# amidos2006/gym-pcgrl

Measured on AMD Instinct MI355X. Metric: env-steps/sec (whole node), binary-narrow 14x14 @ 65536 envs, higher is better.
Workload: dtype u8; 1 GPU; binary-narrow-v0 14x14, 65536 envs/GPU; envs_per_gpu=65536, width=14, height=14, max_changes=39, actions=uniform random, device-generated before the timed region, parallelism=env-axis shard x1, no collective on the step path

## Files before the change

gym_pcgrl_amd/csrc/kernels_stats.h:

```cpp
#pragma once
template <class MaskT>
__device__ __forceinline__ MaskT row_valid(int lane, int W, int H) {
    MaskT full = (W >= (int)(8 * sizeof(MaskT))) ? ~(MaskT)0 : (((MaskT)1 << W) - 1);
    return lane < H ? full : (MaskT)0;
}

template <int PROB = -1>
__device__ __forceinline__ bool finalize_item(const PcgrlParams& P, const DevBufs& B, int e, const int32_t* s,
                                              int mode, int parity, int shard, bool push_reset = true, int rst_list = WL_RST,
                                              const int2* pre = nullptr, const double* reward_pre = nullptr) {
    const int prob = PROB >= 0 ? PROB : P.prob;
    int32_t* st = B.stats + (size_t)e * 8;
    int32_t* start = B.start_stats + (size_t)e * 8;
    if (mode == MODE_STEP) {
        int32_t old[PCGRL_MAX_STATS], sv[PCGRL_MAX_STATS];
        for (int k = 0; k < 8; k++) { old[k] = st[k]; sv[k] = start[k]; }
        const int2 c = pre ? *pre : reinterpret_cast<const int2*>(B.counters)[e];
        const double r = reward_pre ? *reward_pre : compute_reward(P, s, old, prob);
        const bool d = episode_over(P, s, sv, prob) || c.y >= P.max_changes || c.x >= P.max_iterations;
        B.reward[e] = r;
        B.done[e] = d ? 1 : 0;
        episode_account(B, e, r, d);
        int32_t* inf = B.info + (size_t)e * 10;
#pragma unroll
// ... 48 lines not shown
        int32_t* park = (mode == MODE_STEP) ? B.info + (size_t)e * 10 : B.stats + (size_t)e * 8;
        for (int k = 0; k < 8; k++) park[k] = s[k];
        wl_push(B, parity, park_list >= 0 ? park_list : (mode == MODE_STEP ? WL_SOL : WL_SOL2), shard, e);
        return false;
    }
    return finalize_item<PROB>(P, B, e, s, mode, parity, shard, push_reset, WL_RST, nullptr, reward_pre);
}

template <int J>
__device__ __forceinline__ double dpp_down(double v) {
    const long long b = __double_as_longlong(v);
    const int lo = __builtin_amdgcn_update_dpp(0, (int)b, 0x100 + J, 0xF, 0xF, true), hi = __builtin_amdgcn_update_dpp(0, (int)(b >> 32), 0x100 + J, 0xF, 0xF, true);
    return __longlong_as_double(((long long)hi << 32) | (unsigned)lo);
}
__device__ __forceinline__ void zelda_reward_tab(const PcgrlParams& P, ZeldaRewardTab* T) {
    T->w[0] = P.rewards[0]; T->w[1] = P.rewards[1]; T->w[2] = P.rewards[2]; T->w[3] = P.rewards[4]; T->w[4] = P.rewards[3];
    T->w[5] = P.rewards[5]; T->w[6] = P.rewards[6]; T->w[7] = 0.0;
    T->lo[0] = 1; T->lo[1] = 1; T->lo[2] = 1; T->lo[3] = 2; T->lo[4] = 1; T->lo[5] = P.target_enemy_dist; T->lo[6] = PCGRL_IPOS; T->lo[7] = 0;
    T->hi[0] = 1; T->hi[1] = 1; T->hi[2] = 1; T->hi[3] = P.max_enemies; T->hi[4] = 1; T->hi[5] = PCGRL_IPOS; T->hi[6] = PCGRL_IPOS; T->hi[7] = 0;
}
__device__ __forceinline__ double zelda_reward_lanes(const ZeldaRewardTab* T, const int32_t* old, const int32_t* s, int k) {
    const int s0 = s[0], s1 = s[1], s2 = s[2], s3 = s[3], s4 = s[4], s5 = s[5], s6 = s[6];
    int n = s6;
    n = k == 5 ? s5 : n; n = k == 4 ? s4 : n; n = k == 3 ? s3 : n; n = k == 2 ? s2 : n; n = k == 1 ? s1 : n; n = k == 0 ? s0 : n;
    const int kk = k & 7;
    const int o = old[kk];
    const double t = k < 7 ? (double)range_reward_i(n, o, T->lo[kk], T->hi[kk]) * T->w[kk] : 0.0;
    double r = t;
    r = r + dpp_down<1>(t); r = r + dpp_down<2>(t); r = r + dpp_down<3>(t);
    r = r + dpp_down<4>(t); r = r + dpp_down<5>(t); r = r + dpp_down<6>(t);
    return r;
}

template <int PROB, int G, class MaskT, bool FUSED = false>
__device__ __forceinline__ void stats_wave_task(const PcgrlParams& P, const DevBufs& B, DevGroup<G, MaskT>& g, int lane64, int gw, bool lone,
                                                bool inc, bool pair, bool zinc, bool have, int raw, int shard, int mode, int parity,
                                                int inline_reset, int gen_map, uint32_t* mt, uint8_t* tiles, MaskT rowmask,
                                                StepLocal* SL = nullptr, bool step_obs = false) {
    constexpr bool kCanReset = PROB == PCGRL_PROB_BINARY || PROB == PCGRL_PROB_ZELDA;
    if (!kCanReset) inline_reset = 0;
    constexpr int GPW = 64 / G;
    constexpr bool kInc = PROB == PCGRL_PROB_BINARY;
    constexpr bool kZinc = PROB == PCGRL_PROB_ZELDA && G == 16 && sizeof(MaskT) == 4;
    constexpr int NPL = (PROB == PCGRL_PROB_BINARY) ? 1 : 3;
    MaskT* champ_base = reinterpret_cast<MaskT*>(B.champ);
    const bool tch = kInc && G == 16 && !inc && !lone && have && raw < 0;
    const bool packed = inc || (kZinc && zinc && !lone) || tch;
    const bool reset_only = have && !packed && (raw & WL_RESET_ONLY) != 0;
    const bool compute = have && !reset_only && !(lone && (gw & 1));
    const int e = packed ? wl_inc_env<G>(raw) : (raw & ~WL_RESET_ONLY);
    MaskT* planes_e = reinterpret_cast<MaskT*>(B.planes) + (size_t)e * NPL * G;
    MaskT b0 = 0, b1 = 0, b2 = 0;
    if (compute) {
        b0 = planes_e[g.lane * NPL];
        if (NPL > 1) { b1 = planes_e[g.lane * NPL + 1]; b2 = planes_e[g.lane * NPL + 2]; }
    }
    if (GPW >= 2 && lone && inline_reset) {
        const int role = gw & 1;
        int2 pre = make_int2(0, 0);
        if (g.lane == 0 && role == 0 && have) pre = reinterpret_cast<const int2*>(B.counters)[e];
        asm volatile("s_waitcnt vmcnt(0)" ::: "memory");
#pragma unroll
        for (int k = 0; k < GPW / 2; k++) {
            if (k > 0 && !pair) break;
            if (!__builtin_amdgcn_readlane((int)have, 2 * k * G)) continue;
            const int ek = __builtin_amdgcn_readlane(e, 2 * k * G);
            const int step_draws = (SL && P.rep == PCGRL_REP_NARROW && P.random_tile) ? 1 : 0;
            if (SL && lane64 == 0) SL->dirty[ek - SL->e0] = 1;
            ResetRows rr;
            wave_reset_env<PROB, !FUSED, FUSED>(P, B, ek, gen_map, mt, (uint8_t*)nullptr, lane64, step_draws, gw == 2 * k + 1 ? g.lane : -1, &rr);
            MaskT t0, t1, t2;
// ... 48 lines not shown
    } else {
        bool full = compute;
        if (kInc && G == 16) {
            const bool t = compute && tch;
            if (t) {
                const MaskT cbit = (g.lane == wl_inc_row<G>(raw)) ? (MaskT)1 << wl_inc_col<G>(raw) : (MaskT)0;
                const MaskT champ_old = champ_base[(size_t)e * G + g.lane];
                const int4 old = *reinterpret_cast<const int4*>(B.stats + (size_t)e * 8);
                int regions, path, ub2;
                if (binary_touch(g, (MaskT)(~b0 & rowmask), cbit, (wl_inc_code<G>(raw) & 1u) != 0, old.x, champ_old, old.w - 1, regions, path, champ, ub2)) {
                    s[0] = regions; s[1] = path; s[2] = 1; s[3] = ub2 + 1;
                    full = false;
                }
            }
        }
        if (full) need_solver = compute_item_stats<PROB>(g, P, b0, b1, b2, rowmask, s, champ, (B.step_tight & 1) != 0);
    }
    if (kInc && compute && champ_base) champ_base[(size_t)e * G + g.lane] = champ;
    TL(10);
    int want_reset = 0;
    constexpr bool kLaneReward = PROB == PCGRL_PROB_ZELDA && G == 16;
    double rpre = 0.0;
    const bool lane_reward = kLaneReward && SL != nullptr && mode == MODE_STEP;
    if (lane_reward && have && !reset_only) rpre = zelda_reward_lanes(&SL->zr, B.stats + (size_t)e * 8, s, g.lane);
    if (g.lane == 0 && have) {
        if (reset_only) want_reset = 1;
        else want_reset = finish_or_park<PROB>(P, B, e, s, need_solver, mode, parity, shard, !inline_reset, -1, lane_reward ? &rpre : nullptr) ? 1 : 0;
    }
    if (inline_reset) {
        const uint64_t want = __ballot(want_reset != 0);
        TL(11);
        if (want) {
            TL(12);
            if (SL) { while (__hip_atomic_load(&SL->refill_done[SL->par], __ATOMIC_ACQUIRE, __HIP_MEMORY_SCOPE_WORKGROUP) < SL->need) __builtin_amdgcn_s_sleep(2); }
            bool mine = false;
#pragma unroll
            for (int k = 0; k < GPW; k++) {
                if ((want >> (k * G)) & 1ull) {
                    const int ek = __builtin_amdgcn_readlane(e, k * G);
                    if (SL && lane64 == 0) { SL->dirty[ek - SL->e0] = 1; SL->late[ek - SL->e0] = 1; SL->n_late = 1; }
                    int pend = 0;
                    if (SL) {
                        if (lane64 == 0) {
                            pend = atomicExch(&SL->pend[ek - SL->e0], 0);
                            if (pend < 0) {
                                while (__hip_atomic_load(&SL->late_done[(ek - SL->e0) >> 6], __ATOMIC_ACQUIRE, __HIP_MEMORY_SCOPE_WORKGROUP) == 0) __builtin_amdgcn_s_sleep(2);
                                pend = 0;
                            }
                        }
                        pend = __builtin_amdgcn_readfirstlane(pend);
                    }
                    ResetRows rr;
                    wave_reset_env<PROB, !FUSED, FUSED>(P, B, ek, gen_map, mt, (uint8_t*)nullptr, lane64, 0, gw == k ? g.lane : -1, &rr, pend);
                    MaskT t0, t1, t2;
                    reset_rows_to_planes<MaskT>(P, reinterpret_cast<MaskT*>(B.planes) + (size_t)ek * NPL * G, gw == k ? g.lane : -1, rr.m0, rr.m1, rr.m2, t0, t1, t2);
                    if (gw == k) { b0 = t0; b1 = t1; b2 = t2; mine = true; }
                    __builtin_amdgcn_wave_barrier();
                }
            }
            if (mine) {
                int32_t st[PCGRL_MAX_STATS] = {0, 0, 0, 0, 0, 0, 0, 0};
                const bool ns = compute_item_stats<PROB>(g, P, b0, b1, b2, rowmask, st, champ, (B.step_tight & 2) != 0);
                if (kInc && champ_base) champ_base[(size_t)e * G + g.lane] = champ;
                if (g.lane == 0) finish_or_park<PROB>(P, B, e, st, ns, MODE_START, parity, shard);
            }
        }
    }
// ... 316 lines not shown
```

gym_pcgrl_amd/csrc/kernels_step.h:

```cpp
#pragma once

struct StepLds { int planes, champ, stats, start, cnt, cur, fifo, tag, pos, act, flat, in_total, info, rew, done, total; };
__host__ __device__ constexpr StepLds step_lds_layout(int plane_row_bytes, int champ_row_bytes, bool fifo, int action_width, int epb) {
    StepLds L = {};
    int o = 0;
    L.planes = o; o += epb * plane_row_bytes;
    L.champ = o; o += epb * champ_row_bytes;
    L.stats = o; o += epb * 32;
    L.start = o; o += epb * 32;
    L.cnt = o; o += epb * 8;
    L.cur = o; o += epb * 8;
    L.fifo = o; o += fifo ? epb * PCGRL_FIFO_N * 4 : 0;
    L.tag = o; o += fifo ? epb * 4 : 0;
    L.pos = o; o += epb * 2;
    L.act = o; o += epb * 4 * action_width;
    L.flat = o; o += action_width == 3 ? epb * 4 : 0;
    L.in_total = o;
    L.info = o; o += epb * 40;
    L.rew = o; o += epb * 8;
    L.done = o; o += epb;
    L.total = (o + 15) & ~15;
    return L;
}

// ... 129 lines not shown
            PCGRL_SEG_LOAD(L.tag / 16, EPB / 4, has_fifo ? Bg.fifo_tag + e0 : nullptr, has_fifo);
        }
        PCGRL_SEG_LOAD(L.pos / 16, EPB / 8, Bg.pos + (size_t)e0 * 2, true);
        if (!ROW) PCGRL_SEG_LOAD(L.act / 16, EPB / 4 * AW, actions + (size_t)e0 * AW, !(AW == 3 && Bg.flat));
        if (!ROW && AW == 3) PCGRL_SEG_LOAD(L.flat / 16, (AW == 3 ? EPB / 4 : 1), Bg.flat ? Bg.flat + e0 : nullptr, Bg.flat != nullptr);
        asm volatile("" ::: "memory");
        static_assert(L.act % 16 == 0, "the prefetch ends on a slot boundary in front of the actions");
        constexpr int TOT = (ROW ? L.act : L.in_total) / 16;
        seg_store_c<TPB, 0, TOT>(smem, r0, tid0); seg_store_c<TPB, 1, TOT>(smem, r1, tid0); seg_store_c<TPB, 2, TOT>(smem, r2, tid0);
        seg_store_c<TPB, 3, TOT>(smem, r3, tid0); seg_store_c<TPB, 4, TOT>(smem, r4, tid0); seg_store_c<TPB, 5, TOT>(smem, r5, tid0);
        seg_store_c<TPB, 6, TOT>(smem, r6, tid0); seg_store_c<TPB, 7, TOT>(smem, r7, tid0); seg_store_c<TPB, 8, TOT>(smem, r8, tid0);
    } else {
        blk_copy<TPB>(smem + L.planes, g_planes, ne * kPlaneRow);
        if (has_champ) blk_copy<TPB>(smem + L.champ, g_champ, ne * champ_row);
        blk_copy<TPB>(smem + L.stats, reinterpret_cast<const uint8_t*>(Bg.stats + (size_t)e0 * 8), ne * 32);
        blk_copy<TPB>(smem + L.start, reinterpret_cast<const uint8_t*>(Bg.start_stats + (size_t)e0 * 8), ne * 32);
        blk_copy<TPB>(smem + L.cnt, reinterpret_cast<const uint8_t*>(Bg.counters + (size_t)e0 * 2), ne * 8);
        blk_copy<TPB>(smem + L.cur, reinterpret_cast<const uint8_t*>(Bg.rng_cur + (size_t)e0 * 2), ne * 8);
        blk_copy<TPB>(smem + L.pos, Bg.pos + (size_t)e0 * 2, ne * 2);
        if (has_fifo) {
            blk_copy<TPB>(smem + L.fifo, reinterpret_cast<const uint8_t*>(Bg.fifo + (size_t)e0 * PCGRL_FIFO_N), ne * PCGRL_FIFO_N * 4);
            blk_copy<TPB>(smem + L.tag, reinterpret_cast<const uint8_t*>(Bg.fifo_tag + e0), ne * 4);
        }
        if (ROW) {}
        else if (AW == 3 && Bg.flat) blk_copy<TPB>(smem + L.flat, reinterpret_cast<const uint8_t*>(Bg.flat + e0), ne * 4);
        else blk_copy<TPB>(smem + L.act, reinterpret_cast<const uint8_t*>(actions + (size_t)e0 * AW), ne * 4 * AW);
    }
    if (row_have) {
        reinterpret_cast<int32_t*>(smem + (row_fl ? L.flat : L.act))[threadIdx.x] = (int32_t)row_act;
        if (Bg.row.actions_out) Bg.row.actions_out[row_a0] = row_act;
    }
    if (threadIdx.x < EPB) { s_loc.dirty[threadIdx.x] = 0; if (OBS) { s_loc.obs_skip[threadIdx.x] = 0; s_loc.late[threadIdx.x] = 0; } }
    if (threadIdx.x < 8) s_n[threadIdx.x >> 2][threadIdx.x & 3] = 0;
    if (threadIdx.x == 0) { s_loc.e0 = 0; s_loc.need = NUPD; s_loc.refill_done[0] = 0; s_loc.refill_done[1] = 0; s_loc.n_late = 0; s_obs_ticket = 0; }
    constexpr int OBS_PER_TASK = 8;
    const bool obs_delta = OBS && REP == PCGRL_REP_WIDE && NPL == 3 && Bg.obs.delta;
    const int n_obs = (OBS && !obs_delta) ? (ne + OBS_PER_TASK - 1) / OBS_PER_TASK : 0;
    const ObsPlanes<MaskT, NPL> obs_src = {reinterpret_cast<const MaskT*>(smem + L.planes), G};
    if (OBS && threadIdx.x == 0) s_loc.obs_v = obs_view(P, Bg.obs, e0);
    if (PROB == PCGRL_PROB_ZELDA && threadIdx.x == 64) zelda_reward_tab(P, &s_loc.zr);
    uint8_t* reset_scratch = smem + L.total;
#pragma clang loop unroll(disable)
  for (int t = 0; t < (MULTI ? steps : 1); t++) {
    int tid = (int)threadIdx.x;
    if (MULTI) asm volatile("" : "+v"(tid));
    const int lane64 = tid & 63, wv = tid >> 6, gw = lane64 / G;
    const int sp = t & 1;
    DevGroup<G, MaskT> g(lane64);
    if (MULTI && t > 0) {
        const int32_t* row = actions + (size_t)t * action_stride + (size_t)e0 * AW;
        for (int i = tid; i < ne * AW; i += TPB) reinterpret_cast<int32_t*>(smem + L.act)[i] = row[i];
    }
    __syncthreads();
    TL(17);
    const int prio = B.step_prio, prio_nfull = (prio >> 8) & 15;
    int prio_now = 0;
    if (wv < NUPD) {
        if ((prio >> 6) & 3) { prio_now = (prio >> 6) & 3; step_set_prio(prio_now); }
        const int e = wv * 64 + lane64;
        UpdateOut u = {};
        UpdateMid mid = {};
        if (REP == PCGRL_REP_WIDE && !MULTI && Bg.flat && e < ne) {
            const int dim = P.ntiles, total = W * H * dim;
            int a = reinterpret_cast<const int32_t*>(smem + L.flat)[e];
            if (a < 0 || a >= total) atomicOr(B.status, PCGRL_STATUS_BAD_ACTION);
            a = a < 0 ? 0 : (a >= total ? total - 1 : a);
            int32_t* t3 = reinterpret_cast<int32_t*>(smem + L.act) + 3 * e;
            const int q = a / dim;
            t3[0] = q % W; t3[1] = q / W; t3[2] = a - q * dim;
        }
        if (e < ne) u = update_env<REP, MaskT, true, true, true>(P, B, act_lds, e, &mid);
        TL(2);
        const bool first = u.rst || u.sure_done;
        const bool packed_full = PROB == PCGRL_PROB_ZELDA && B.zelda_inc;
        int dest = -1, v = e;
        if (first) { dest = 0; v = u.rst ? (e | WL_RESET_ONLY) : e; }
        else if (u.chg) { dest = u.cheap ? 2 : 1; v = (u.cheap || packed_full) ? u.inc_item : ((u.touch && B.step_touch) ? (u.inc_item | (int)0x80000000) : e); }
        if (u.chg) s_loc.dirty[e] = 1;
        if (OBS && first && e < EPB) s_loc.obs_skip[e] = 1;
        const uint64_t m0 = __ballot(dest == 0), m1 = __ballot(dest == 1), m2 = __ballot(dest == 2);
        const uint64_t below = (1ull << lane64) - 1ull;
        int b0 = 0, b1 = 0, b2 = 0;
        if (lane64 == 0) {
            b0 = m0 ? atomicAdd(&s_n[sp][0], __popcll(m0)) : 0;
            b1 = m1 ? atomicAdd(&s_n[sp][1], __popcll(m1)) : 0;
            b2 = m2 ? atomicAdd(&s_n[sp][2], __popcll(m2)) : 0;
            if (wv == 0) { s_n[sp ^ 1][0] = 0; s_n[sp ^ 1][1] = 0; s_n[sp ^ 1][2] = 0; s_n[sp ^ 1][3] = 0; s_loc.refill_done[sp ^ 1] = 0; s_loc.par = sp; }
        }
        b0 = __builtin_amdgcn_readfirstlane(b0); b1 = __builtin_amdgcn_readfirstlane(b1); b2 = __builtin_amdgcn_readfirstlane(b2);
        if (dest == 0) s_items[0][b0 + __popcll(m0 & below)] = v;
        if (dest == 2) s_items[2][b2 + __popcll(m2 & below)] = v;
        {
            const int lvl = (u.bucket >> 3) & 7;
            int pos1 = 0;
#pragma unroll
            for (int b = 0; b < 8; b++) {
                const uint64_t mb = __ballot(dest == 1 && lvl == b);
                pos1 += b > lvl ? __popcll(mb) : (b == lvl ? __popcll(mb & below) : 0);
            }
            if (dest == 1) s_items[1][b1 + pos1] = v;
        }
        asm volatile("s_waitcnt lgkmcnt(0)" ::: "memory");
        __builtin_amdgcn_s_barrier();
        int k_used = 0, cur0 = 0;
        if (lane64 == 0) s_loc.late_done[wv] = 0;
        if (e < ne && !first) update_env_cursor<REP, MaskT>(P, B, e, mid, k_used, cur0);
        if (OBS && REP == PCGRL_REP_WIDE && NPL == 3 && obs_delta && e < ne && !first && u.chg) obs_write_delta_piece(obs_src, obs_view_from_lds(&s_loc.obs_v), e, act_lds[3 * e], act_lds[3 * e + 1]);
        if (e < EPB) s_loc.pend[e] = (has_fifo && e < ne && !first) ? k_used : 0;
        asm volatile("s_waitcnt vmcnt(0) lgkmcnt(0)" ::: "memory");
        if (lane64 == 0) __hip_atomic_fetch_add(&s_loc.refill_done[sp], 1, __ATOMIC_RELEASE, __HIP_MEMORY_SCOPE_WORKGROUP);
    }
    int n0 = 0, n1 = 0, n2 = 0, w_full = 0, w_total = 0, w_lone = 0;
    bool stats_left = true, obs_left = OBS;
    bool pair = false;
    const int fpw = B.step_fpw, ipw = B.step_ipw;
    const int tiles_bytes = (W * H + 15) & ~15;
    uint32_t* mt = reinterpret_cast<uint32_t*>(reset_scratch + (size_t)wv * (PCGRL_MT_N * 4 + tiles_bytes));
    uint8_t* tiles = reinterpret_cast<uint8_t*>(mt + PCGRL_MT_N);
    const MaskT rowmask = row_valid<MaskT>(g.lane, W, H);
    const bool zinc = PROB == PCGRL_PROB_ZELDA && sizeof(MaskT) == 4 && B.zelda_inc;
    for (bool first_round = true;; first_round = false) {
        if (first_round) {
            if (wv >= NUPD) {
                asm volatile("s_waitcnt lgkmcnt(0)" ::: "memory");
                __builtin_amdgcn_s_barrier();
                asm volatile("" ::: "memory");
            }
            TL(3);
            n0 = s_n[sp][0]; n1 = s_n[sp][1]; n2 = s_n[sp][2];
            w_full = (n1 + fpw - 1) / fpw;
            pair = PROB == PCGRL_PROB_ZELDA && B.step_pair > 0 && n0 >= B.step_pair;
            w_lone = pair ? (n0 + 1) >> 1 : n0;
            w_total = w_lone + w_full + (n2 + ipw - 1) / ipw;
        }
        if (OBS && !first_round && obs_left) {
            int oid = 0;
            if (lane64 == 0) oid = atomicAdd(&s_obs_ticket, 1);
            oid = __builtin_amdgcn_readfirstlane(oid);
            if (oid >= n_obs) obs_left = false;
            else {
                if (prio_now) { prio_now = 0; step_set_prio(0); }
                while (__hip_atomic_load(&s_loc.refill_done[sp], __ATOMIC_ACQUIRE, __HIP_MEMORY_SCOPE_WORKGROUP) < NUPD) __builtin_amdgcn_s_sleep(2);
                const int o0 = oid * OBS_PER_TASK;
                const ObsView V = obs_view_from_lds(&s_loc.obs_v);
#pragma clang loop unroll(disable)
                for (int j = 0; j < OBS_PER_TASK; j++) {
                    const int eo = o0 + j;
                    if (eo < ne && !s_loc.obs_skip[eo]) obs_write_env_lean(obs_src, V, smem + L.pos, eo, lane64);
                }
            }
        }
        if (!stats_left) { if (!OBS || !obs_left) break; continue; }
        int wid = 0;
        if (lane64 == 0) wid = atomicAdd(&s_n[sp][3], 1);
        wid = __builtin_amdgcn_readfirstlane(wid);
        TL(18);
        if (wid >= w_total) { stats_left = false; if (!OBS || !obs_left) break; continue; }
        const bool lone = wid < w_lone, inc = wid >= w_lone + w_full;
        const int item = lone ? (pair ? 2 * wid + (gw >> 1) : wid) : (inc ? (wid - w_lone - w_full) * ipw + gw : (wid - w_lone) * fpw + gw);
        const bool have = lone ? (item < n0 && (pair || gw < 2)) : (gw < (inc ? ipw : fpw) && item < (inc ? n2 : n1));
        const int raw = have ? s_items[lone ? 0 : (inc ? 2 : 1)][item] : 0;
        TL(lone ? 4 : (inc ? 6 : 5));
        if (prio) {
            const int want = lone ? (prio & 3) : (inc ? ((prio >> 4) & 3) : ((prio_nfull == 0 || wid - w_lone < prio_nfull) ? ((prio >> 2) & 3) : 0));
            if (want != prio_now) { prio_now = want; step_set_prio(want); }
        }
        stats_wave_task<PROB, G, MaskT, true>(P, B, g, lane64, gw, lone, inc, PROB == PCGRL_PROB_ZELDA && pair, zinc, have, raw, lane64, MODE_STEP, parity, 1, gen_map, mt, tiles, rowmask, &s_loc, OBS);
        TL(7);
    }
    if (prio_now) { prio_now = 0; step_set_prio(0); }
    if (has_fifo && wv < NUPD) {
        const int e = wv * 64 + lane64;
        int k = 0;
        if (e < ne) k = atomicExch(&s_loc.pend[e], -1);
        if (k > 0) {
            int c0 = B.rng_cur[2 * e] - k;
            c0 = c0 < 0 ? c0 + PCGRL_MT_N : c0;
            fifo_refill(B, e, k, c0);
        }
        asm volatile("s_waitcnt vmcnt(0) lgkmcnt(0)" ::: "memory");
        if (lane64 == 0) __hip_atomic_store(&s_loc.late_done[wv], 1, __ATOMIC_RELEASE, __HIP_MEMORY_SCOPE_WORKGROUP);
    }
    TL(8);
    if (MULTI && (reward_out || done_out || info_out)) {
        __syncthreads();
        const size_t row = (size_t)t * P.num_envs + e0;
        if (reward_out && tid < ne) reward_out[row + tid] = reinterpret_cast<const double*>(smem + L.rew)[tid];
        if (done_out && tid >= TPB / 2 && tid - TPB / 2 < ne) done_out[row + tid - TPB / 2] = smem[L.done + tid - TPB / 2];
        if (info_out) for (int i = tid; i < ne * 10; i += TPB) info_out[row * 10 + i] = reinterpret_cast<const int32_t*>(smem + L.info)[i];
    }
  }
    __syncthreads();
    blk_copy<TPB>(reinterpret_cast<uint8_t*>(Bg.stats + (size_t)e0 * 8), smem + L.stats, ne * 32);
    blk_copy<TPB>(reinterpret_cast<uint8_t*>(Bg.info + (size_t)e0 * 10), smem + L.info, ne * 40);
    blk_copy<TPB>(reinterpret_cast<uint8_t*>(Bg.reward + e0), smem + L.rew, ne * 8);
    blk_copy<TPB>(reinterpret_cast<uint8_t*>(Bg.counters + (size_t)e0 * 2), smem + L.cnt, ne * 8);
    blk_copy<TPB>(reinterpret_cast<uint8_t*>(Bg.rng_cur + (size_t)e0 * 2), smem + L.cur, ne * 8);
    blk_copy<TPB>(Bg.pos + (size_t)e0 * 2, smem + L.pos, ne * 2);
    blk_copy<TPB>(Bg.done + e0, smem + L.done, ne);
    if (has_fifo) {
        blk_copy<TPB>(reinterpret_cast<uint8_t*>(Bg.fifo + (size_t)e0 * PCGRL_FIFO_N), smem + L.fifo, ne * PCGRL_FIFO_N * 4);
        blk_copy<TPB>(reinterpret_cast<uint8_t*>(Bg.fifo_tag + e0), smem + L.tag, ne * 4);
// ... 34 lines not shown
```

gym_pcgrl_amd/csrc/pcgrl_abi.hip:

```cpp
#include <hip/hip_runtime.h>
#include <stdio.h>
#include <stdlib.h>
#include <string.h>

#include <vector>

#include "../../include/pcgrl_hip.h"

#ifdef PCGRL_PART
#define PCGRL_IN_PART(k) (PCGRL_PART == (k))
#else
#define PCGRL_IN_PART(k) 1
#endif
#define PCGRL_LOCAL __attribute__((visibility("hidden")))
#define PART_CORE 0
#define PART_STATS 1
#define PART_UPDATE 2
#define PART_STEP_BINARY 3
#define PART_STEP_ZELDA 4
#define PART_SEARCH 5
#define PART_SMB 6
#define PART_STEP_SOLVER 7

#include "lanegroup_dev.h"
// ... 309 lines not shown
    if (!b->map || !b->old_map || !b->heatmap || !b->pos || !b->planes || !b->counters || !b->stats ||
        !b->start_stats || !b->info || !b->reward || !b->done || !b->tile_p || !b->rng_rep || !b->rng_cursor || !b->scratch)
        return PCGRL_EINVAL;
    if (h->cfg.prob == PCGRL_BINARY && !b->rng_prob) return PCGRL_EINVAL;
    {
        hipPointerAttribute_t at;
        if (hipPointerGetAttributes(&at, b->map) == hipSuccess) h->device = at.device;
        else { (void)hipGetLastError(); HIPCHK(hipGetDevice(&h->device)); }
    }
    DeviceGuard guard(h->device);
    int rc0 = device_setup(h);
    if (rc0) return rc0;
    const pcgrl_tuning& T = h->tun;
    h->no_wide = tun_or(T.no_wide, 0) ? 1 : 0;
    h->wide_waves = tun_or(T.wide_waves, 8);
    h->wide_pairs = tun_or(T.wide_pairs, 1);
    h->wide_grid = tun_or(T.wide_grid, 2048);
    if (h->wide_grid < 1) h->wide_grid = 2048;
    h->fused_zelda = tun_or(T.fused_zelda, 1) ? 1 : 0;
    h->no_fused = tun_or(T.no_fused, 0) ? 1 : 0;
    h->obs_at_end = tun_or(T.obs_at_end, 0) ? 1 : 0;
    h->async_split = tun_or(T.async_split, h->cfg.prob == PCGRL_SOKOBAN ? 1 : 0) ? 1 : 0;
    {
        const int n_ = h->cfg.num_envs;
        h->step_epb = T.step_epb > 0 ? T.step_epb : ((n_ >= 192 * 256 && n_ <= 256 * 256) ? 256 : (n_ >= 192 * 128 ? 128 : 64));
        if (h->step_epb != 128 && h->step_epb != 256) h->step_epb = 64;
        h->smb_heap = T.smb_lds_heap > 0 ? T.smb_lds_heap : SMB_LDS_HEAP;
        if (h->smb_heap < 256 || h->smb_heap > 4096) h->smb_heap = SMB_LDS_HEAP;
    }
    {
        const int f = tun_or(T.full_per_wave, 4), i = tun_or(T.inc_per_wave, 4);
        h->B.step_fpw = (f == 1 || f == 2) ? f : 4;
        h->B.step_prio = tun_or(T.step_prio, h->cfg.prob == PCGRL_BINARY ? (h->cfg.rep == PCGRL_NARROW ? (15 | (3 << 6)) : 15) : 0) & 0xFFF;
        h->B.step_ipw = (i == 1 || i == 2) ? i : 4;
        h->B.step_touch = tun_or(T.no_touch, 0) ? 0 : 1;
        h->B.step_pair = tun_or(T.step_pair, 6);
        h->B.step_tight = h->B.step_touch ? tun_or(T.touch_tight, 1) : 0;
    }
    const bool no_inc = tun_or(T.no_inc, 0) != 0;
    DevBufs& B = h->B;
    B.map = (uint8_t*)b->map; B.old_map = (uint8_t*)b->old_map; B.heat = (uint16_t*)b->heatmap; B.pos = (uint8_t*)b->pos;
    B.heat_end = B.heat + (size_t)h->cfg.num_envs * h->cfg.width * h->cfg.height;
    B.heat32 = h->cfg.auto_reset ? 0 : 1;
    B.ep_return = nullptr; B.ep_length = nullptr; B.last_return = nullptr; B.last_length = nullptr;
    B.local = nullptr;
    B.planes = b->planes; B.counters = (int32_t*)b->counters; B.stats = (int32_t*)b->stats;
    B.start_stats = (int32_t*)b->start_stats; B.info = (int32_t*)b->info; B.reward = (double*)b->reward;
    B.done = (uint8_t*)b->done; B.tile_p = (double*)b->tile_p; B.rng_rep = (uint32_t*)b->rng_rep;
    B.rng_prob = (uint32_t*)b->rng_prob; B.rng_cur = (int32_t*)b->rng_cursor;
    uint8_t* s = (uint8_t*)b->scratch;
    B.wl_cnt = (int32_t*)s;
    B.status = (int32_t*)(s + WL_CNT_BYTES);
    {
        uint8_t* q = s + WL_CNT_BYTES + 256;
        for (int k = 0; k < WL_NLIST; k++) {
            B.wl_cap[k] = wl_capacity(h->cfg.num_envs, k);
            B.wl_items[k] = (int32_t*)q;
            q += wl_list_bytes(h->cfg.num_envs, k);
        }
    }
    HIPCHK(hipMemsetAsync(B.wl_cnt, 0, WL_CNT_BYTES + 256, (hipStream_t)stream));
    B.sok_pool = nullptr; B.sok_heap = nullptr; B.sok_table = nullptr;
    B.zelda_inc = (h->cfg.prob == PCGRL_ZELDA && h->cfg.rep <= PCGRL_REP_TURTLE && h->cfg.height <= 16 && h->cfg.width <= 32 &&
                   h->cfg.num_envs <= WL_INC_ENV_MASK && !no_inc) ? 1 : 0;
    B.pair_min = tun_or(T.pair_min, 2048);
    B.big_team = tun_or(T.big_team, 1) ? 1 : 0;
// ... 1051 lines not shown
```

gym_pcgrl_amd/csrc/pcgrl_algos.h:

```cpp
#pragma once
#include "pcgrl_common.h"

#if defined(__HIPCC__) && defined(__HIP_DEVICE_COMPILE__)
#define PCGRL_NO_IFCVT() asm volatile("" ::: "memory")
#else
#define PCGRL_NO_IFCVT() do {} while (0)
#endif
#ifndef PCGRL_TRACE
#define PCGRL_TRACE(g, site)
#endif

struct PcgrlParams {
    int32_t prob, rep, num_envs, width, height, ntiles, nplanes, group, mask_bytes;
    int32_t max_changes, max_iterations;
    int32_t random_start, random_tile, warp, random_probs, auto_reset;
    int32_t target_path, max_enemies, target_enemy_dist, max_crates, target_solution, solver_power;
    int32_t prob_width, prob_height;
    int32_t max_potions, max_treasures;
    int32_t max_diamonds, min_spikes, target_jumps;
    int32_t min_empty, min_enemies, min_jumps;
    int32_t big, big_search;
    double target_col_enemies;
    double rewards[PCGRL_MAX_REWARDS];
    double cdf[PCGRL_MAX_TILES];
// ... 304 lines not shown
#ifdef PCGRL_EXP_NOSWEEP
    return g.popcount_sum(comp) / 4 + 1;
#endif
    typename B::mask_t last, unused;
    const int e1 = bfs_levels(g, g.first_bit(comp), comp, last);
    if (2 * e1 <= best) return 0;
    return bfs_levels<false>(g, g.first_bit(last), comp, unused);
}

template <class B>
PCGRL_D void regions_and_longest_path(B& g, typename B::mask_t pass, int& regions, int& path, typename B::mask_t& champ, int& ub2, bool tight = true) {
    typedef typename B::mask_t M;
    regions = 0;
    path = 0;
    ub2 = -1;
    champ = pass ^ pass;
    const M nontiny = pass & ~pcg_tiny_components(g, pass, regions, path);
    if (!g.any(nontiny)) return;
    const PcgFillCtx<B> ctx = pcg_fill_ctx(g, pass);
    if (B::kGroup != 16) {
        typedef typename B::ivec_t I;
        M rest = nontiny;
        const I cnt = g.popc_lanes(rest);
        M seed = g.first_bit(g.keep_where_eq(cnt, g.imax(cnt), rest));
        while (g.any(rest)) {
            const M comp = pcg_component(g, seed, ctx);
            rest = rest & ~comp;
            ++regions;
            if (g.popcount_sum(comp) - 1 > path) { const int e = pcg_double_sweep(g, comp, path); if (e > path) { path = e; champ = comp; } }
            seed = g.first_bit(rest);
        }
        return;
    }
    M rest = nontiny, big1 = nontiny ^ nontiny, big2 = big1;
    int size1 = 0, size2 = 0, size3 = 0;
    while (g.any(rest)) {
        const M comp = pcg_component(g, g.first_bit(rest), ctx);
        rest = rest & ~comp;
        ++regions;
        const int size = g.popcount_sum(comp);
        if (size > size1) { size3 = size2; size2 = size1; big2 = big1; size1 = size; big1 = comp; }
        else if (size > size2) { size3 = size2; size2 = size; big2 = comp; }
        else if (size > size3) size3 = size;
    }
    const int tiny_path = path;
    int bd1 = size1 - 1, bd2 = size2 - 1, who = 0;
    if (size1 - 1 > path) { const int e = pcg_double_sweep(g, big1, path, bd1); if (e > path) { path = e; champ = big1; who = 1; } }
    {
        const int rest_b = size3 - 1 > tiny_path ? size3 - 1 : tiny_path;
        if (size2 - 1 > path) { const int e = pcg_double_sweep(g, big2, path, bd2); if (e > path) { path = e; champ = big2; who = 2; } }
        else if (tight && size2 - 1 > rest_b) pcg_double_sweep(g, big2, rest_b, bd2);
    }
    if (size3 - 1 > path) {
        rest = nontiny & ~big1 & ~big2;
        while (g.any(rest)) {
            const M comp = pcg_component(g, g.first_bit(rest), ctx);
            rest = rest & ~comp;
            if (g.popcount_sum(comp) - 1 > path) { const int e = pcg_double_sweep(g, comp, path); if (e > path) { path = e; champ = comp; who = 3; } }
        }
    }
    const int b1 = who == 1 ? 0 : bd1, b2 = who == 2 ? 0 : bd2, b3 = size3 - 1;
    ub2 = tiny_path;
    ub2 = b1 > ub2 ? b1 : ub2; ub2 = b2 > ub2 ? b2 : ub2; ub2 = b3 > ub2 ? b3 : ub2;
    ub2 = ub2 > path ? path : ub2;
}
template <class B>
PCGRL_D void regions_and_longest_path(B& g, typename B::mask_t pass, int& regions, int& path, typename B::mask_t& champ) {
    int ub2;
    regions_and_longest_path(g, pass, regions, path, champ, ub2);
}
template <class B>
PCGRL_D void regions_and_longest_path(B& g, typename B::mask_t pass, int& regions, int& path) {
    typename B::mask_t champ;
    regions_and_longest_path(g, pass, regions, path, champ);
}

template <class B>
PCGRL_D void binary_incremental(B& g, typename B::mask_t pass_new, typename B::mask_t cbit, bool added, int regions_old, int path_old,
                                typename B::mask_t champ_old, int ub2_old, int& regions, int& path, typename B::mask_t& champ, int& ub2) {
    typedef typename B::mask_t M;
    const M base = pass_new & ~cbit;
    M rest = pcg_neighbours(g, cbit) & base;
    path = path_old;
    champ = champ_old;
    constexpr bool kTrack = B::kGroup == 16;
    const bool track = kTrack && ub2_old >= 0;
    int k = 0, ub = track ? ub2_old : 0;
    M uni = cbit;
    if (g.any(rest)) {
        const PcgFillCtx<B> ctx = pcg_fill_ctx(g, base);
        while (g.any(rest)) {
// ... 269 lines not shown
```

gym_pcgrl_amd/csrc/worklist.h:

```cpp
#pragma once
#define PCGRL_BLOCK 256
#define PCGRL_STATUS_TOO_MANY_CRATES 1
#define PCGRL_STATUS_BAD_ACTION 2
#define PCGRL_STATUS_BAD_TILE 4
enum { MODE_STEP = 0, MODE_START = 1, MODE_SETMAP = 2 };

#define WL_NSHARD 64
#define WL_WIDE_FEW_REGIONS 32
#define WL_CSTRIDE 16
enum { WL_CHG = 0, WL_RST = 1, WL_SOL = 2, WL_SOL2 = 3, WL_RST2 = 4, WL_SOL3 = 5, WL_INC = 6, WL_NLIST = 7 };
#ifndef SMB_LONG_POPS
#define SMB_LONG_POPS 2000
#endif
#define WL_INC_ENV_MASK 0x1FFFFF
#define WL_INC64_ENV_MASK 0x7FFFF
__device__ __forceinline__ int wl_inc_pack(int group, int e, int row, int col, unsigned code) {
    return group == 16 ? (int)((unsigned)e | ((unsigned)(row * 32 + col) << 21) | (code << 30))
                       : (int)((unsigned)e | ((unsigned)(row * 64 + col) << 19) | ((code & 1u) << 31));
}
#define WL_INCBIG_ENV_MASK 0x7FFF
__device__ __forceinline__ int wl_incbig_pack(int e, int x, int y, bool added) { return (int)((unsigned)e | ((unsigned)x << 15) | ((unsigned)y << 23) | (added ? 0x80000000u : 0u)); }
template <int G> __device__ __forceinline__ int wl_inc_env(int raw) { return raw & (G == 16 ? WL_INC_ENV_MASK : WL_INC64_ENV_MASK); }
template <int G> __device__ __forceinline__ int wl_inc_row(int raw) { return G == 16 ? ((raw >> 26) & 15) : ((raw >> 25) & 63); }
template <int G> __device__ __forceinline__ int wl_inc_col(int raw) { return G == 16 ? ((raw >> 21) & 31) : ((raw >> 19) & 63); }
// ... 39 lines not shown
    int32_t wide_spin;
    int32_t wide_few;
    int32_t wide_epoch;
    const uint16_t* heat_end;
    double* ep_return; int32_t* ep_length; double* last_return; int32_t* last_length;
    int32_t* counters; int32_t* stats; int32_t* start_stats; int32_t* info;
    double* reward; uint8_t* done; double* tile_p;
    uint32_t* rng_rep; uint32_t* rng_prob; int32_t* rng_cur;
    int32_t* wl_cnt;
    int32_t* wl_items[WL_NLIST];
    int32_t wl_cap[WL_NLIST];
    SokNode* sok_pool; uint32_t* sok_heap; uint32_t* sok_table; int32_t* status;
    int32_t* sok_res;
    int32_t* sok_cnt; int32_t* sok_stop;
    struct LocalLists* local;
    int32_t md_only_agent;
    int32_t* sok_sync;
    int32_t sok_pool_stride, sok_heap_stride, sok_table_size, sok_use_lds;
    int32_t sok_spawn_iters;
    int32_t sok_hard_cap;
    int32_t sok_fast_maxc;
    int32_t inline_reset;
    int32_t pair_min;
    int32_t zelda_inc;
    uint32_t* fifo; int32_t* fifo_tag;
    ObsSpec obs;
    int32_t step_fpw, step_ipw;
    int32_t step_prio;
    int32_t step_tight;
    const int32_t* flat;
    int32_t step_pair;
    int32_t big_team;
    int32_t step_touch;
    uint8_t* big_arena;
    uint8_t* pending; unsigned long long* async_stats;
    const uint8_t* async_slots; size_t async_slot_bytes; int32_t async_nslots; int32_t* async_run; int32_t* async_run_n;
    int32_t heat32;
    RowBind row; int32_t act_i64;
};
#define PCGRL_FIFO_N 8

struct ZeldaRewardTab { double w[8]; int lo[8]; int hi[8]; };
struct ObsView {
    uint8_t* out;
    int oh, ow, depth, centered, pad, W, H;
};
struct StepLocal {
    int e0;
    int par, need;
    int refill_done[2];
    int pend[256];
    int late_done[4];
    uint8_t dirty[256];
    uint8_t obs_skip[256];
    uint8_t late[256];
    int n_late;
    ObsView obs_v;
    ZeldaRewardTab zr;
};

__device__ __forceinline__ void async_list_runnable(const DevBufs& B, int gi) {
    if (gi < B.async_nslots && __hip_atomic_load(reinterpret_cast<const int32_t*>(B.async_slots + (size_t)gi * B.async_slot_bytes), __ATOMIC_RELAXED, __HIP_MEMORY_SCOPE_AGENT) == 1)
        B.async_run[atomicAdd(B.async_run_n, 1)] = gi;
}
__device__ __forceinline__ int32_t* wl_counters(const DevBufs& B, int parity, int list) {
    return B.wl_cnt + (size_t)(parity * WL_NLIST + list) * WL_NSHARD * WL_CSTRIDE;
}
#define WL_LOCAL_CAP 512
struct LocalLists { int n[WL_NLIST]; int e0; uint16_t items[WL_NLIST][WL_LOCAL_CAP]; };
__device__ __forceinline__ void wl_push(const DevBufs& B, int parity, int list, int shard, int value) {
    if (B.local) {
        const int i = atomicAdd(&B.local->n[list], 1);
        B.local->items[list][i] = (uint16_t)(value - B.local->e0);
        return;
    }
    const int i = atomicAdd(wl_counters(B, parity, list) + shard * WL_CSTRIDE, 1);
    B.wl_items[list][(size_t)shard * B.wl_cap[list] + i] = value;
}
__device__ __forceinline__ int wl_load_prefix(const DevBufs& B, int parity, int list, int* s_pref) {
    if (threadIdx.x < WL_NSHARD) {
        int v = wl_counters(B, parity, list)[threadIdx.x * WL_CSTRIDE];
        for (int o = 1; o < WL_NSHARD; o <<= 1) {
            const int t = __shfl_up(v, o, 64);
// ... 165 lines not shown
```

Before: 2.296 billion env-steps/s.

## Defer refill publish until a reset needs it and track third-largest component

Each update wave used to wait for all outstanding memory ops and publish refill_done right after its cursor update. That publish is now deferred by default and happens only when a reset actually needs it, or after the wave's stats task, so waves move straight into stats work. A separate cursor_done counter lets observation tasks wait on LDS writes alone. Separately, the longest-path search now tracks a third-largest component and sweeps it directly before scanning the rest, with tie handling intended to keep champion selection identical. This adds complexity to the intra-block synchronisation protocol and a risk of ordering bugs.

New measurement: 2.310 billion env-steps/s (median of 6 runs). About the same (+0.6%).

```diff
diff --git a/gym_pcgrl_amd/csrc/kernels_stats.h b/gym_pcgrl_amd/csrc/kernels_stats.h
--- a/gym_pcgrl_amd/csrc/kernels_stats.h
+++ b/gym_pcgrl_amd/csrc/kernels_stats.h
@@ -104,11 +104,17 @@
     return r;
 }
 
+__device__ __forceinline__ void step_publish(StepLocal* SL, int lane64, bool& unpublished) {
+    asm volatile("s_waitcnt vmcnt(0) lgkmcnt(0)" ::: "memory");
+    if (lane64 == 0) __hip_atomic_fetch_add(&SL->refill_done[SL->par], 1, __ATOMIC_RELEASE, __HIP_MEMORY_SCOPE_WORKGROUP);
+    unpublished = false;
+}
+
 template <int PROB, int G, class MaskT, bool FUSED = false>
 __device__ __forceinline__ void stats_wave_task(const PcgrlParams& P, const DevBufs& B, DevGroup<G, MaskT>& g, int lane64, int gw, bool lone,
                                                 bool inc, bool pair, bool zinc, bool have, int raw, int shard, int mode, int parity,
                                                 int inline_reset, int gen_map, uint32_t* mt, uint8_t* tiles, MaskT rowmask,
-                                                StepLocal* SL = nullptr, bool step_obs = false) {
+                                                StepLocal* SL = nullptr, bool step_obs = false, bool* unpublished = nullptr) {
     constexpr bool kCanReset = PROB == PCGRL_PROB_BINARY || PROB == PCGRL_PROB_ZELDA;
     if (!kCanReset) inline_reset = 0;
     constexpr int GPW = 64 / G;
@@ -223,7 +229,10 @@
         TL(11);
         if (want) {
             TL(12);
-            if (SL) { while (__hip_atomic_load(&SL->refill_done[SL->par], __ATOMIC_ACQUIRE, __HIP_MEMORY_SCOPE_WORKGROUP) < SL->need) __builtin_amdgcn_s_sleep(2); }
+            if (SL) {
+                if (FUSED && unpublished && *unpublished) step_publish(SL, lane64, *unpublished);
+                while (__hip_atomic_load(&SL->refill_done[SL->par], __ATOMIC_ACQUIRE, __HIP_MEMORY_SCOPE_WORKGROUP) < SL->need) __builtin_amdgcn_s_sleep(2);
+            }
             bool mine = false;
 #pragma unroll
             for (int k = 0; k < GPW; k++) {
diff --git a/gym_pcgrl_amd/csrc/kernels_step.h b/gym_pcgrl_amd/csrc/kernels_step.h
--- a/gym_pcgrl_amd/csrc/kernels_step.h
+++ b/gym_pcgrl_amd/csrc/kernels_step.h
@@ -185,7 +185,7 @@
     }
     if (threadIdx.x < EPB) { s_loc.dirty[threadIdx.x] = 0; if (OBS) { s_loc.obs_skip[threadIdx.x] = 0; s_loc.late[threadIdx.x] = 0; } }
     if (threadIdx.x < 8) s_n[threadIdx.x >> 2][threadIdx.x & 3] = 0;
-    if (threadIdx.x == 0) { s_loc.e0 = 0; s_loc.need = NUPD; s_loc.refill_done[0] = 0; s_loc.refill_done[1] = 0; s_loc.n_late = 0; s_obs_ticket = 0; }
+    if (threadIdx.x == 0) { s_loc.e0 = 0; s_loc.need = NUPD; s_loc.refill_done[0] = 0; s_loc.refill_done[1] = 0; s_loc.cursor_done[0] = 0; s_loc.cursor_done[1] = 0; s_loc.n_late = 0; s_obs_ticket = 0; }
     constexpr int OBS_PER_TASK = 8;
     const bool obs_delta = OBS && REP == PCGRL_REP_WIDE && NPL == 3 && Bg.obs.delta;
     const int n_obs = (OBS && !obs_delta) ? (ne + OBS_PER_TASK - 1) / OBS_PER_TASK : 0;
@@ -208,6 +208,7 @@
     TL(17);
     const int prio = B.step_prio, prio_nfull = (prio >> 8) & 15;
     int prio_now = 0;
+    bool unpublished = false;
     if (wv < NUPD) {
         if ((prio >> 6) & 3) { prio_now = (prio >> 6) & 3; step_set_prio(prio_now); }
         const int e = wv * 64 + lane64;
@@ -238,7 +239,7 @@
             b0 = m0 ? atomicAdd(&s_n[sp][0], __popcll(m0)) : 0;
             b1 = m1 ? atomicAdd(&s_n[sp][1], __popcll(m1)) : 0;
             b2 = m2 ? atomicAdd(&s_n[sp][2], __popcll(m2)) : 0;
-            if (wv == 0) { s_n[sp ^ 1][0] = 0; s_n[sp ^ 1][1] = 0; s_n[sp ^ 1][2] = 0; s_n[sp ^ 1][3] = 0; s_loc.refill_done[sp ^ 1] = 0; s_loc.par = sp; }
+            if (wv == 0) { s_n[sp ^ 1][0] = 0; s_n[sp ^ 1][1] = 0; s_n[sp ^ 1][2] = 0; s_n[sp ^ 1][3] = 0; s_loc.refill_done[sp ^ 1] = 0; s_loc.cursor_done[sp ^ 1] = 0; s_loc.par = sp; }
         }
         b0 = __builtin_amdgcn_readfirstlane(b0); b1 = __builtin_amdgcn_readfirstlane(b1); b2 = __builtin_amdgcn_readfirstlane(b2);
         if (dest == 0) s_items[0][b0 + __popcll(m0 & below)] = v;
@@ -260,8 +261,12 @@
         if (e < ne && !first) update_env_cursor<REP, MaskT>(P, B, e, mid, k_used, cur0);
         if (OBS && REP == PCGRL_REP_WIDE && NPL == 3 && obs_delta && e < ne && !first && u.chg) obs_write_delta_piece(obs_src, obs_view_from_lds(&s_loc.obs_v), e, act_lds[3 * e], act_lds[3 * e + 1]);
         if (e < EPB) s_loc.pend[e] = (has_fifo && e < ne && !first) ? k_used : 0;
-        asm volatile("s_waitcnt vmcnt(0) lgkmcnt(0)" ::: "memory");
-        if (lane64 == 0) __hip_atomic_fetch_add(&s_loc.refill_done[sp], 1, __ATOMIC_RELEASE, __HIP_MEMORY_SCOPE_WORKGROUP);
+        if (OBS) {
+            asm volatile("s_waitcnt lgkmcnt(0)" ::: "memory");
+            if (lane64 == 0) __hip_atomic_fetch_add(&s_loc.cursor_done[sp], 1, __ATOMIC_RELEASE, __HIP_MEMORY_SCOPE_WORKGROUP);
+        }
+        unpublished = true;
+        if (!B.step_early) step_publish(&s_loc, lane64, unpublished);
     }
     int n0 = 0, n1 = 0, n2 = 0, w_full = 0, w_total = 0, w_lone = 0;
     bool stats_left = true, obs_left = OBS;
@@ -293,7 +298,7 @@
             if (oid >= n_obs) obs_left = false;
             else {
                 if (prio_now) { prio_now = 0; step_set_prio(0); }
-                while (__hip_atomic_load(&s_loc.refill_done[sp], __ATOMIC_ACQUIRE, __HIP_MEMORY_SCOPE_WORKGROUP) < NUPD) __builtin_amdgcn_s_sleep(2);
+                while (__hip_atomic_load(&s_loc.cursor_done[sp], __ATOMIC_ACQUIRE, __HIP_MEMORY_SCOPE_WORKGROUP) < NUPD) __builtin_amdgcn_s_sleep(2);
                 const int o0 = oid * OBS_PER_TASK;
                 const ObsView V = obs_view_from_lds(&s_loc.obs_v);
 #pragma clang loop unroll(disable)
@@ -318,9 +323,11 @@
             const int want = lone ? (prio & 3) : (inc ? ((prio >> 4) & 3) : ((prio_nfull == 0 || wid - w_lone < prio_nfull) ? ((prio >> 2) & 3) : 0));
             if (want != prio_now) { prio_now = want; step_set_prio(want); }
         }
-        stats_wave_task<PROB, G, MaskT, true>(P, B, g, lane64, gw, lone, inc, PROB == PCGRL_PROB_ZELDA && pair, zinc, have, raw, lane64, MODE_STEP, parity, 1, gen_map, mt, tiles, rowmask, &s_loc, OBS);
+        stats_wave_task<PROB, G, MaskT, true>(P, B, g, lane64, gw, lone, inc, PROB == PCGRL_PROB_ZELDA && pair, zinc, have, raw, lane64, MODE_STEP, parity, 1, gen_map, mt, tiles, rowmask, &s_loc, OBS, &unpublished);
+        if (unpublished) step_publish(&s_loc, lane64, unpublished);
         TL(7);
     }
+    if (unpublished) step_publish(&s_loc, lane64, unpublished);
     if (prio_now) { prio_now = 0; step_set_prio(0); }
     if (has_fifo && wv < NUPD) {
         const int e = wv * 64 + lane64;
diff --git a/gym_pcgrl_amd/csrc/pcgrl_abi.hip b/gym_pcgrl_amd/csrc/pcgrl_abi.hip
--- a/gym_pcgrl_amd/csrc/pcgrl_abi.hip
+++ b/gym_pcgrl_amd/csrc/pcgrl_abi.hip
@@ -365,6 +365,7 @@
         const int f = tun_or(T.full_per_wave, 4), i = tun_or(T.inc_per_wave, 4);
         h->B.step_fpw = (f == 1 || f == 2) ? f : 4;
         h->B.step_prio = tun_or(T.step_prio, h->cfg.prob == PCGRL_BINARY ? (h->cfg.rep == PCGRL_NARROW ? (15 | (3 << 6)) : 15) : 0) & 0xFFF;
+        h->B.step_early = (T.step_prio >= 0 && (T.step_prio & 0x1000)) ? 0 : 1;
         h->B.step_ipw = (i == 1 || i == 2) ? i : 4;
         h->B.step_touch = tun_or(T.no_touch, 0) ? 0 : 1;
         h->B.step_pair = tun_or(T.step_pair, 6);
diff --git a/gym_pcgrl_amd/csrc/pcgrl_algos.h b/gym_pcgrl_amd/csrc/pcgrl_algos.h
--- a/gym_pcgrl_amd/csrc/pcgrl_algos.h
+++ b/gym_pcgrl_amd/csrc/pcgrl_algos.h
@@ -360,16 +360,17 @@
         }
         return;
     }
-    M rest = nontiny, big1 = nontiny ^ nontiny, big2 = big1;
-    int size1 = 0, size2 = 0, size3 = 0;
+    M rest = nontiny, big1 = nontiny ^ nontiny, big2 = big1, big3 = big1;
+    int size1 = 0, size2 = 0, size3 = 0, size4 = 0;
     while (g.any(rest)) {
         const M comp = pcg_component(g, g.first_bit(rest), ctx);
         rest = rest & ~comp;
         ++regions;
         const int size = g.popcount_sum(comp);
-        if (size > size1) { size3 = size2; size2 = size1; big2 = big1; size1 = size; big1 = comp; }
-        else if (size > size2) { size3 = size2; size2 = size; big2 = comp; }
-        else if (size > size3) size3 = size;
+        if (size > size1) { size4 = size3; size3 = size2; big3 = big2; size2 = size1; big2 = big1; size1 = size; big1 = comp; }
+        else if (size > size2) { size4 = size3; size3 = size2; big3 = big2; size2 = size; big2 = comp; }
+        else if (size > size3) { size4 = size3; size3 = size; big3 = comp; }
+        else if (size > size4) size4 = size;
     }
     const int tiny_path = path;
     int bd1 = size1 - 1, bd2 = size2 - 1, who = 0;
@@ -380,11 +381,17 @@
         else if (tight && size2 - 1 > rest_b) pcg_double_sweep(g, big2, rest_b, bd2);
     }
     if (size3 - 1 > path) {
-        rest = nontiny & ~big1 & ~big2;
-        while (g.any(rest)) {
-            const M comp = pcg_component(g, g.first_bit(rest), ctx);
-            rest = rest & ~comp;
-            if (g.popcount_sum(comp) - 1 > path) { const int e = pcg_double_sweep(g, comp, path); if (e > path) { path = e; champ = comp; who = 3; } }
+        bool tie = false;
+        { const int e = pcg_double_sweep(g, big3, path); if (e > path) { path = e; champ = big3; who = 3; tie = true; } }
+        if (size4 - 1 > (tie ? path - 1 : path)) {
+            rest = nontiny & ~big1 & ~big2 & ~big3;
+            while (g.any(rest)) {
+                const M comp = pcg_component(g, g.first_bit(rest), ctx);
+                rest = rest & ~comp;
+                const bool ahead = tie && g.any(g.first_bit(comp | big3) & comp);
+                const int thr = ahead ? path - 1 : path;
+                if (g.popcount_sum(comp) - 1 > thr) { const int e = pcg_double_sweep(g, comp, thr); if (e > thr) { path = e; champ = comp; who = 3; tie = false; } }
+            }
         }
     }
     const int b1 = who == 1 ? 0 : bd1, b2 = who == 2 ? 0 : bd2, b3 = size3 - 1;
diff --git a/gym_pcgrl_amd/csrc/worklist.h b/gym_pcgrl_amd/csrc/worklist.h
--- a/gym_pcgrl_amd/csrc/worklist.h
+++ b/gym_pcgrl_amd/csrc/worklist.h
@@ -95,6 +95,7 @@
     int32_t step_pair;
     int32_t big_team;
     int32_t step_touch;
+    int32_t step_early;
     uint8_t* big_arena;
     uint8_t* pending; unsigned long long* async_stats;
     const uint8_t* async_slots; size_t async_slot_bytes; int32_t async_nslots; int32_t* async_run; int32_t* async_run_n;
@@ -112,6 +113,7 @@
     int e0;
     int par, need;
     int refill_done[2];
+    int cursor_done[2];
     int pend[256];
     int late_done[4];
     uint8_t dirty[256];
```
